# JoernZheng/parallel-data-compression-and-decompression

Hardware: NVIDIA B200
Metric: deflate/inflate GB/s (uncompressed) (higher is better)
Workload: dtype u8

## Files before the change

### parallel-data-compression-and-decompression_b200/csrc/deflate_match.cuh

```cuda
#pragma once
#include "zwz_common.cuh"

namespace zwz {

#define ZWZ_DM_NIL 0xffffu
#ifndef ZWZ_DM_NOISE_BITS
#define ZWZ_DM_NOISE_BITS 7.7f
#endif

#ifdef ZWZ_EMU
static uint64_t g_dm_stats[4];
extern "C" void zwz_emu_match_stats(uint64_t *out, int reset) {
    for (int i = 0; i < 4; ++i) {
        out[i] = g_dm_stats[i];
        if (reset) g_dm_stats[i] = 0;
    }
}
#define ZWZ_DM_STAT(i, v) do { g_dm_stats[i] += (v); } while (0)
#else
#define ZWZ_DM_STAT(i, v) do { } while (0)
#endif

template <int CLS> struct MatchClass;
template <> struct MatchClass<0> {
    static constexpr uint32_t kCap = 8192, kThreads = 256, kHBits = 12, kData = 8192 + 64, kListBits = 3, kCtasPerSm = 6;
    static constexpr uint32_t kPrevBytes = ((kCap + 31u) & ~31u) * 2u, kSmem = kData + kPrevBytes + (2u << kHBits) + 1024u + 2u * 8u * 8u;
};
template <> struct MatchClass<1> {
    static constexpr uint32_t kCap = 16384, kThreads = 512, kHBits = 13, kData = 16384 + 64, kListBits = 4, kCtasPerSm = 3;
    static constexpr uint32_t kPrevBytes = ((kCap + 31u) & ~31u) * 2u, kSmem = kData + kPrevBytes + (2u << kHBits) + 1024u + 2u * 16u * 16u;
};
template <> struct MatchClass<2> {
    static constexpr uint32_t kCap = 31744, kThreads = 512, kHBits = 13, kData = 31744 + 64, kListBits = 4, kCtasPerSm = 2;
    static constexpr uint32_t kPrevBytes = ((kCap + 31u) & ~31u) * 2u, kSmem = kData + kPrevBytes + (2u << kHBits) + 1024u + 2u * 16u * 16u;
};
template <> struct MatchClass<3> {
    static constexpr uint32_t kCap = 65535, kThreads = 1024, kHBits = 14, kData = 65600, kListBits = 5, kCtasPerSm = 1;
    static constexpr uint32_t kPrevBytes = ((kCap + 31u) & ~31u) * 2u, kSmem = kData + kPrevBytes + (2u << kHBits) + 640u + 2u * 32u * 32u;
};

struct MatchCtl {
    unsigned long long mbar;
    uint32_t next_tile;
    uint32_t cur_work;
    uint32_t nmatch;
    uint32_t skip[2];
    uint32_t coll;
    uint32_t coll2;
    uint32_t set2;
    uint32_t base[33];
    uint32_t adler_a[32], adler_b[32], adler_len[32];
};
static_assert(sizeof(MatchCtl) <= 640, "MatchCtl must fit its slot");
static_assert(MatchClass<0>::kPrevBytes >= (2u << MatchClass<0>::kHBits) && MatchClass<1>::kPrevBytes >= (2u << MatchClass<1>::kHBits) &&
                  MatchClass<2>::kPrevBytes >= (2u << MatchClass<2>::kHBits) && MatchClass<3>::kPrevBytes >= (2u << MatchClass<3>::kHBits),
              "the second bit set of the noise test lives in prev[]");
static_assert(2u * (MatchClass<2>::kSmem + 1024u) <= 228u * 1024u && 3u * (MatchClass<1>::kSmem + 1024u) <= 228u * 1024u &&
                  6u * (MatchClass<0>::kSmem + 1024u) <= 228u * 1024u,
              "resident CTAs per SM assumed by the launch grids");

ZWZ_DEV uint32_t dm_scratch_match_words(uint32_t n) { return scr_match_words(n); }

template <int HBITS> ZWZ_DEV uint32_t dm_hash3(uint32_t b0, uint32_t b1, uint32_t b2) {
    uint32_t v = b0 | (b1 << 8) | (b2 << 16);
    return (v * 0x9E3779B1u) >> (32 - HBITS);
}

#ifndef ZWZ_EMU
ZWZ_DEV uint32_t dm_smem_addr(const void *p) { return (uint32_t) __cvta_generic_to_shared(p); }
ZWZ_DEV void dm_mbar_init(unsigned long long *bar) {
    asm volatile("mbarrier.init.shared::cta.b64 [%0], 1;" ::"r"(dm_smem_addr(bar)));
    asm volatile("fence.mbarrier_init.release.cluster;" ::: "memory");
}
ZWZ_DEV void dm_bulk_g2s(void *dst, const void *src, uint32_t bytes, unsigned long long *bar) {
    asm volatile("fence.proxy.async.shared::cta;" ::: "memory");
    asm volatile("mbarrier.arrive.expect_tx.shared::cta.b64 _, [%0], %1;" ::"r"(dm_smem_addr(bar)), "r"(bytes) : "memory");
    asm volatile("cp.async.bulk.shared::cluster.global.mbarrier::complete_tx::bytes [%0], [%1], %2, [%3];" ::"r"(dm_smem_addr(dst)),
                 "l"(src), "r"(bytes), "r"(dm_smem_addr(bar))
                 : "memory");
}
ZWZ_DEV void dm_mbar_wait(unsigned long long *bar, uint32_t parity) {
    uint32_t done = 0;
    while (!done) {
        asm volatile("{\n\t.reg .pred p;\n\tmbarrier.try_wait.parity.shared::cta.b64 p, [%1], %2;\n\tselp.u32 %0, 1, 0, p;\n\t}"
                     : "=r"(done)
                     : "r"(dm_smem_addr(bar)), "r"(parity)
                     : "memory");
    }
}
#endif

ZWZ_DEV uint32_t sD_of(const unsigned char *smem, uint32_t skew) { return smem_addr(smem) + skew; }

template <int CLS, bool DICT = false>
ZWZ_KERNEL __launch_bounds__(MatchClass<CLS>::kThreads, MatchClass<CLS>::kCtasPerSm) lz_match_kernel(DeflateJob job, const uint32_t *__restrict__ order, uint32_t n_work,
                                                                         uint32_t *work_counter) {
    constexpr uint32_t T = MatchClass<CLS>::kThreads, HB = MatchClass<CLS>::kHBits, DATA = MatchClass<CLS>::kData;
    constexpr uint32_t NW = T / 32u, LB = MatchClass<CLS>::kListBits;
    static_assert((1u << LB) == NW, "one position list per warp");
    ZWZ_DYN_SMEM(smem);
    const uint32_t *dataw = (const uint32_t *) smem;
    uint16_t *prev = (uint16_t *) (smem + DATA);
    uint16_t *head = (uint16_t *) (smem + DATA + MatchClass<CLS>::kPrevBytes);
    MatchCtl *ctl = (MatchCtl *) (smem + DATA + MatchClass<CLS>::kPrevBytes + (2u << HB));
    uint16_t *cnt = (uint16_t *) ((unsigned char *) ctl + 640);
    const uint8_t *datab = (const uint8_t *) smem;
    const unsigned tid = threadIdx.x, lane = lane_id(), wid = warp_id();
    const unsigned lt = (1u << lane) - 1u;
    uint32_t parity = 0;

#ifndef ZWZ_EMU
    if (tid == 0) dm_mbar_init(&ctl->mbar);
#endif
    __syncthreads();

    for (;;) {
        if (tid == 0) ctl->cur_work = atomicAdd(work_counter, 1u);
        __syncthreads();
        const uint32_t w = ctl->cur_work;
        if (w >= n_work) break;
        const uint32_t c = order[w];
        const uint32_t n = job.raw_len[c];
        const uint8_t *src = job.raw + job.raw_off[c];
        const uint32_t skew = (uint32_t) ((uintptr_t) src & 15u);
        const uint32_t stage_bytes = (skew + n + 15u) & ~15u;
        const uint8_t *drec = nullptr;
        uint32_t dwl = 0;
        if (DICT) {
            const uint32_t di = job.dict.idx[c];
            if (di != ZWZ_NO_DICT) {
                drec = job.dict.arena + (size_t) di * ZWZ_DICT_STRIDE;
                dwl = job.dict.wlen[di];
            }
        }

#ifndef ZWZ_EMU
        if (tid == 0 && stage_bytes) dm_bulk_g2s(smem, src - skew, stage_bytes, &ctl->mbar);
#else
        for (uint32_t i = tid; i < skew + n; i += T) smem[i] = i < skew ? 0 : src[i - skew];
#endif
        for (uint32_t i = tid; i < NW * NW / 2u; i += T) ((uint32_t *) cnt)[i] = 0u;
        if (tid == 0) {
            ctl->next_tile = 0;
            ctl->nmatch = 0;
            ctl->skip[0] = 0;
            ctl->skip[1] = 0;
        }
#ifndef ZWZ_EMU
        if (stage_bytes) dm_mbar_wait(&ctl->mbar, parity);
        parity ^= (stage_bytes != 0u);
#endif
        __syncthreads();
        if (tid < 32u) smem[skew + n + tid] = 0;

        {
            uint32_t *hist = (uint32_t *) head + wid * 256u;
            const uint32_t nfull = n >> 10;
            for (uint32_t kb = wid; kb < nfull; kb += NW) {
                const uint32_t w0 = (skew + (kb << 10)) >> 2;
                {
                    const uint32_t sv = dataw[w0 + 8u * lane] & 0x80808080u;
                    const uint32_t tops = (uint32_t) (__popc(__ballot_sync(ZWZ_FULL, sv & 0x80u)) + __popc(__ballot_sync(ZWZ_FULL, sv & 0x8000u)) +
                                                      __popc(__ballot_sync(ZWZ_FULL, sv & 0x800000u)) + __popc(__ballot_sync(ZWZ_FULL, sv & 0x80000000u)));
                    if (tops < 40u || tops > 88u) continue;
                }
#pragma unroll
                for (uint32_t j = 0; j < 8u; ++j) hist[lane + 32u * j] = 0u;
                __syncwarp();
#pragma unroll
                for (uint32_t j = 0; j < 8u; ++j) {
                    const uint32_t wv = dataw[w0 + lane + 32u * j];
                    atomicAdd(&hist[wv & 0xffu], 1u);
                    atomicAdd(&hist[(wv >> 8) & 0xffu], 1u);
                    atomicAdd(&hist[(wv >> 16) & 0xffu], 1u);
                    atomicAdd(&hist[wv >> 24], 1u);
                }
                __syncwarp();
                float sum = 0.f;
#pragma unroll
                for (uint32_t j = 0; j < 8u; ++j) {
                    const float cf = (float) hist[lane + 32u * j];
                    if (cf > 1.f) sum += cf * zwz_log2f(cf);
                }
#pragma unroll
                for (int d = 16; d > 0; d >>= 1) sum += __shfl_xor_sync(ZWZ_FULL, sum, d);
                if (lane == 0 && sum < (10.f - ZWZ_DM_NOISE_BITS) * 1024.f) atomicOr(&ctl->skip[kb >> 5], 1u << (kb & 31u));
                __syncwarp();
            }
            __syncthreads();
            const uint64_t cand = (uint64_t) ctl->skip[0] | ((uint64_t) ctl->skip[1] << 32);
            if (cand) {
                constexpr uint32_t BB = HB + 4u;
                uint32_t *bits = (uint32_t *) head;
                __syncthreads();
                uint32_t *bits2 = (uint32_t *) prev;
                for (uint32_t i = tid; i < (1u << BB) / 32u; i += T) {
                    bits[i] = 0u;
                    bits2[i] = 0u;
                }
                if (tid == 0) {
                    ctl->coll = 0;
                    ctl->coll2 = 0;
                    ctl->set2 = 0;
                }
                __syncthreads();
                uint32_t mine = 0;
                for (uint32_t st = wid; st < nfull * 32u; st += NW) {
                    if (!((cand >> (st >> 5)) & 1ull)) continue;
                    const uint32_t h = (lds32u(sD_of(smem, skew) + st * 32u + lane) * 0x9E3779B1u) >> (32u - BB);
                    const uint32_t old = atomicOr(&bits[h >> 5], 1u << (h & 31u));
                    mine += (uint32_t) __popc(__ballot_sync(ZWZ_FULL, (old >> (h & 31u)) & 1u));
                }
                if (lane == 0 && mine) atomicAdd(&ctl->coll, mine);
                __syncthreads();
                const uint32_t nh = n >= 3u ? n - 2u : 0u;
                uint32_t fresh = 0;
                for (uint32_t st = wid; st * 32u < nh; st += NW) {
                    if (st < nfull * 32u && ((cand >> (st >> 5)) & 1ull)) continue;
                    const uint32_t q = st * 32u + lane;
                    const uint32_t h = (lds32u(sD_of(smem, skew) + q) * 0x9E3779B1u) >> (32u - BB);
                    const uint32_t old2 = q < nh ? atomicOr(&bits2[h >> 5], 1u << (h & 31u)) : 0xffffffffu;
                    fresh += (uint32_t) __popc(__ballot_sync(ZWZ_FULL, !((old2 >> (h & 31u)) & 1u)));
                }
                if (lane == 0 && fresh) atomicAdd(&ctl->set2, fresh);
                __syncthreads();
                uint32_t hits = 0;
                for (uint32_t st = wid; st < nfull * 32u; st += NW) {
                    if (!((cand >> (st >> 5)) & 1ull)) continue;
                    const uint32_t h = (lds32u(sD_of(smem, skew) + st * 32u + lane) * 0x9E3779B1u) >> (32u - BB);
                    hits += (uint32_t) __popc(__ballot_sync(ZWZ_FULL, (bits2[h >> 5] >> (h & 31u)) & 1u));
                }
                if (lane == 0 && hits) atomicAdd(&ctl->coll2, hits);
                __syncthreads();
                const uint32_t nc = (uint32_t) __popcll((long long) cand) << 10;
                const uint32_t allowed = (uint32_t) (((uint64_t) nc * nc) >> (BB + 1u)) + (nc >> 6) + 48u;
                const uint32_t allowed2 = (uint32_t) (((uint64_t) ctl->set2 * nc) >> BB) + (nc >> 6) + 48u;
                if (tid == 0 && (ctl->coll > allowed || ctl->coll2 > allowed2)) {
                    ctl->skip[0] = 0;
                    ctl->skip[1] = 0;
                    ZWZ_DM_STAT(1, 1);
                }
            }
        }
        __syncthreads();
        for (uint32_t i = tid; i < (1u << HB) / 2u; i += T) ((uint32_t *) head)[i] = 0xffffffffu;
        const uint64_t skipmask = (uint64_t) ctl->skip[0] | ((uint64_t) ctl->skip[1] << 32);
        if (tid == 0) {
            ZWZ_DM_STAT(0, (uint64_t) __popcll((long long) skipmask));
            ZWZ_DM_STAT(2, 1);
        }
        __syncthreads();

        uint32_t *mout = job.scratch + job.scr_off[c];
        uint16_t *list = (uint16_t *) (mout + dm_scratch_match_words(n));
        const uint32_t nhash = n >= 3u ? n - 2u : 0u;
        const uint32_t ntiles = (n + 31u) >> 5;
        const uint32_t nsteps = (nhash + 31u) >> 5;
        const uint32_t spw = (nsteps + NW - 1u) / NW;

        const uint32_t sD = smem_addr(smem) + skew;
        const uint32_t sP = smem_addr(prev);
        const uint32_t sH = smem_addr(head);
        const uint32_t sC = smem_addr(cnt);
        const uint32_t sB = smem_addr(&ctl->base[0]);
        for (uint32_t st = wid * spw; st < (wid + 1u) * spw && st < nsteps; ++st) {
            if ((skipmask >> (st >> 5)) & 1ull) continue;
            const uint32_t p = st * 32u + lane;
            const bool valid = p < nhash;
            uint32_t h = 0;
            if (valid) {
                uint32_t v = lds32u(sD + p);
                h = dm_hash3<HB>(v & 0xffu, (v >> 8) & 0xffu, (v >> 16) & 0xffu);
                sts16(sP + 2u * p, h);
            }
            const uint32_t b = h >> (HB - LB);
            unsigned m = __ballot_sync(ZWZ_FULL, valid);
#pragma unroll
            for (uint32_t k = 0; k < LB; ++k) {
                unsigned v = __ballot_sync(ZWZ_FULL, (b >> k) & 1u);
                m &= ((b >> k) & 1u) ? v : ~v;
            }
            if (valid && (m >> lane) == 1u) sts16(sC + 2u * (wid * NW + b), lds16(sC + 2u * (wid * NW + b)) + (uint32_t) __popc(m));
            __syncwarp();
        }
        __syncthreads();
        if (wid == 0) {
            uint32_t run = 0;
            if (lane < NW) {
                for (uint32_t ww = 0; ww < NW; ++ww) {
                    uint32_t t = cnt[ww * NW + lane];
                    cnt[ww * NW + lane] = (uint16_t) run;
                    run += t;
                }
            }
            uint32_t incl = warp_incl_scan(run);
            if (lane < NW) ctl->base[lane] = incl - run;
            if (lane == NW - 1u) ctl->base[NW] = incl;
        }
        __syncthreads();
        for (uint32_t st = wid * spw; st < (wid + 1u) * spw && st < nsteps; ++st) {
            if ((skipmask >> (st >> 5)) & 1ull) continue;
            const uint32_t p = st * 32u + lane;
            const bool valid = p < nhash;
            const uint32_t h = valid ? lds16(sP + 2u * p) : 0u;
            const uint32_t b = h >> (HB - LB);
            unsigned m = __ballot_sync(ZWZ_FULL, valid);
#pragma unroll
            for (uint32_t k = 0; k < LB; ++k) {
                unsigned v = __ballot_sync(ZWZ_FULL, (b >> k) & 1u);
                m &= ((b >> k) & 1u) ? v : ~v;
            }
            if (valid) {
                uint32_t slot = lds32(sB + 4u * b) + lds16(sC + 2u * (wid * NW + b)) + (uint32_t) __popc(m & lt);
                list[slot] = (uint16_t) p;
            }
            __syncwarp();
            if (valid && (m >> lane) == 1u) sts16(sC + 2u * (wid * NW + b), lds16(sC + 2u * (wid * NW + b)) + (uint32_t) __popc(m));
            __syncwarp();
        }
        __threadfence_block();
        __syncthreads();

        {
            const uint32_t i_end = ctl->base[wid + 1u];
            uint32_t i0 = ctl->base[wid];
            uint32_t qn = (i0 + lane < i_end) ? (uint32_t) __ldcg(list + i0 + lane) : 0u;
            for (; i0 < i_end; i0 += 32u) {
                const bool valid = i0 + lane < i_end;
                const uint32_t q = qn;
                qn = (i0 + 32u + lane < i_end) ? (uint32_t) __ldcg(list + i0 + 32u + lane) : 0u;
                const uint32_t h = valid ? lds16(sP + 2u * q) : 0u;
                uint32_t old = ZWZ_DM_NIL;
                if (valid) old = lds16(sH + 2u * h);
                __syncwarp();
                if (valid) {
                    sts16(sP + 2u * q, old);
                    sts16(sH + 2u * h, q);
                }
                __syncwarp();
                uint32_t rb = valid ? lds16(sH + 2u * h) : q;
                unsigned rem = __ballot_sync(ZWZ_FULL, rb != q);
                while (rem) {
                    const int leader = __ffs((int) rem) - 1;
                    const uint32_t hl = __shfl_sync(ZWZ_FULL, h, leader);
                    const bool mine = valid && h == hl;
                    const unsigned same = __ballot_sync(ZWZ_FULL, mine);
                    const unsigned lower = same & lt;
                    const int from = (mine && lower) ? 31 - __clz((int) lower) : (int) lane;
                    const uint32_t qlow = __shfl_sync(ZWZ_FULL, q, from);
                    if (mine) {
                        if (lower) sts16(sP + 2u * q, qlow);
                        if ((same >> lane) == 1u) sts16(sH + 2u * h, q);
                    }
                    rem &= ~same;
                }
                __syncwarp();
            }
        }
        __syncthreads();
        {
            const uint32_t list_lines = (nhash * 2u + 127u) >> 7;
            for (uint32_t i = tid; i < list_lines; i += T) discard_l2_line((const unsigned char *) list + 128u * i);
        }
        uint32_t *tflags = (uint32_t *) cnt;
        for (uint32_t i = tid; i < ZWZ_SCR_FLAG_WORDS && i < NW * NW / 2u; i += T) tflags[i] = 0u;
        __syncthreads();

        for (;;) {
            uint32_t tile = 0;
            if (lane == 0) tile = atomicAdd(&ctl->next_tile, 1u);
            tile = __shfl_sync(ZWZ_FULL, tile, 0);
            if (tile >= ntiles) break;
            if ((skipmask >> (tile >> 5)) & 1ull) {
                if (lane == 0) atomicMax(&ctl->next_tile, ((tile >> 5) + 1u) << 5);
                continue;
            }

            const uint32_t p = tile * 32u + lane;
            uint32_t best_len = 2u, best_dist = 0u;
            uint32_t maxlen = 0u;
            if (p < nhash) {
                maxlen = (n - p) < ZWZ_MAX_MATCH ? (n - p) : ZWZ_MAX_MATCH;
                const uint32_t limit = p > ZWZ_MAX_DIST ? p - ZWZ_MAX_DIST : 0u;
                const uint32_t span = p - limit;
                uint32_t cand = lds16(sP + 2u * p);
                if ((cand - limit) < span || (DICT && dwl != 0u && p < ZWZ_MAX_DIST)) {
                    const uint32_t ap = sD + p;
                    const uint32_t ka = ap & ~3u, sa = (ap & 3u) * 8u;
                    const uint32_t a0 = lds32(ka), a1 = lds32(ka + 4u), a2 = lds32(ka + 8u), a3 = lds32(ka + 12u);
                    const uint32_t S0 = __funnelshift_r(a0, a1, sa), S1 = __funnelshift_r(a1, a2, sa), S2 = __funnelshift_r(a2, a3, sa);
                    uint32_t scan_end = (S0 >> 16) & 0xffu, scan_end1 = (S0 >> 8) & 0xffu;
                    uint32_t budget = job.depth;
                    for (; budget != 0u && (cand - limit) < span; --budget) {
                        const uint32_t ac = sD + cand;
                        const uint32_t nxt = lds16(sP + 2u * cand);
                        if (lds8(ac + best_len) == scan_end && lds8(ac + best_len - 1u) == scan_end1) {
                            const uint32_t kc = ac & ~3u, sc = (ac & 3u) * 8u;
                            const uint32_t c0 = lds32(kc), c1 = lds32(kc + 4u), c2 = lds32(kc + 8u), c3 = lds32(kc + 12u);
                            const uint32_t x0 = __funnelshift_r(c0, c1, sc) ^ S0, x1 = __funnelshift_r(c1, c2, sc) ^ S1,
                                           x2 = __funnelshift_r(c2, c3, sc) ^ S2;
                            uint32_t len;
                            if (x0) {
                                len = ((uint32_t) __ffs((int) x0) - 1u) >> 3;
                            } else if (x1) {
                                len = 4u + (((uint32_t) __ffs((int) x1) - 1u) >> 3);
                            } else if (x2) {
                                len = 8u + (((uint32_t) __ffs((int) x2) - 1u) >> 3);
                            } else {
                                len = 12u;
                                while (len < maxlen) {
                                    uint32_t y = lds32u(ac + len) ^ lds32u(ap + len);
                                    if (y) {
                                        len += ((uint32_t) __ffs((int) y) - 1u) >> 3;
                                        break;
                                    }
                                    len += 4u;
                                }
                            }
                            if (len > maxlen) len = maxlen;
                            if (len > best_len) {
                                best_len = len;
                                best_dist = p - cand;
                                if (len >= job.nice || len >= maxlen) break;
                                scan_end = lds8(ap + len);
                                scan_end1 = lds8(ap + len - 1u);
                            }
                        }
                        cand = nxt;
                    }
                    if (DICT && budget != 0u && best_len < job.nice && best_len < maxlen && dwl != 0u && p < ZWZ_MAX_DIST) {
                        const uint16_t *dhead = (const uint16_t *) (drec + ZWZ_DICT_HEAD), *dprev = (const uint16_t *) (drec + ZWZ_DICT_PREV);
                        const uint8_t *dwin = drec + ZWZ_DICT_WIN;
                        const uint32_t dlim = p + dwl > ZWZ_MAX_DIST ? p + dwl - ZWZ_MAX_DIST : 0u;
                        const uint32_t dspan = dwl - dlim;
                        uint32_t q = __ldg(dhead + dm_hash3<ZWZ_DICT_HBITS>(S0 & 0xffu, (S0 >> 8) & 0xffu, (S0 >> 16) & 0xffu));
                        for (; budget != 0u && (q - dlim) < dspan; --budget) {
                            const uint32_t nxt = __ldg(dprev + q);
                            const uint32_t dmax = dwl - q < maxlen ? dwl - q : maxlen;
                            if (best_len < dmax && __ldg(dwin + q + best_len) == scan_end && __ldg(dwin + q + best_len - 1u) == scan_end1) {
                                uint32_t len = 0;
                                while (len < dmax) {
                                    const uint32_t y = ld32u((const uint32_t *) dwin, q + len) ^ lds32u(ap + len);
                                    if (y) {
                                        len += ((uint32_t) __ffs((int) y) - 1u) >> 3;
                                        break;
                                    }
                                    len += 4u;
                                }
                                if (len > dmax) len = dmax;
                                if (len > best_len) {
                                    best_len = len;
                                    best_dist = p + dwl - q;
                                    if (len >= job.nice || len >= maxlen) break;
                                    scan_end = lds8(ap + len);
                                    scan_end1 = lds8(ap + len - 1u);
                                }
                            }
                            q = nxt;
                        }
                    }
                }
            }
            if (__any_sync(ZWZ_FULL, best_len >= 4u)) {
                uint32_t key = best_len >= 3u ? best_len + lane : 0u, kd = best_dist;
#pragma unroll
                for (int d = 1; d < 32; d <<= 1) {
                    const uint32_t ok = __shfl_up_sync(ZWZ_FULL, key, d), od = __shfl_up_sync(ZWZ_FULL, kd, d);
                    if (lane >= (unsigned) d && ok > key) {
                        key = ok;
                        kd = od;
                    }
                }
                if (key >= lane + 3u && key - lane > best_len && key - lane <= maxlen) {
                    best_len = key - lane;
                    best_dist = kd;
                }
            }
            if (best_len == 3u && best_dist > 4096u) best_len = 2u;
            const unsigned hit = __ballot_sync(ZWZ_FULL, best_len >= 3u);
            if (hit) {
                if (p < n) mout[p] = tok_make(lds8(sD + p), best_len >= 3u ? best_len : 0u, best_dist);
                if (lane == 0) {
                    atomicAdd(&ctl->nmatch, (uint32_t) __popc(hit));
                    atomicOr(&tflags[tile >> 5], 1u << (tile & 31u));
                }
            }
        }
        __syncthreads();
        {
            uint32_t *gflags = mout + scr_flag_offset(n);
            const uint32_t used = (ntiles + 31u) >> 5;
            for (uint32_t i = tid; i < ZWZ_SCR_FLAG_WORDS; i += T) gflags[i] = i < used ? tflags[i] : 0u;
        }

        {
            AdlerPart part;
            part.a = 0;
            part.b = 0;
            part.len = 0;
            const uint32_t nwords = (skew + n + 3u) >> 2;
            for (uint32_t j = tid; j < nwords; j += T) {
                uint32_t wv = dataw[j];
                const int pos0 = (int) (4u * j) - (int) skew;
                if (pos0 < 0) wv = pos0 <= -4 ? 0u : wv & (0xffffffffu << (8u * (uint32_t) (-pos0)));
                if (pos0 + 4 > (int) n) wv &= 0xffffffffu >> (8u * (uint32_t) (pos0 + 4 - (int) n));
                const uint32_t s4 = zwz_dp4a(wv, 0x01010101u), w4 = zwz_dp4a(wv, 0x03020100u);
                part.a += s4;
                part.b += (uint32_t) ((int) n - pos0) * s4 - w4;
            }
            part.b %= 65521u;
#pragma unroll
            for (int d = 1; d < 32; d <<= 1) {
                AdlerPart o;
                o.a = __shfl_down_sync(ZWZ_FULL, part.a, d);
                o.b = __shfl_down_sync(ZWZ_FULL, part.b, d);
                o.len = __shfl_down_sync(ZWZ_FULL, part.len, d);
                if ((lane & (2u * d - 1u)) == 0u) part = adler_combine(part, o);
            }
            if (lane == 0) {
                ctl->adler_a[wid] = part.a;
                ctl->adler_b[wid] = part.b;
                ctl->adler_len[wid] = part.len;
            }
            __syncthreads();
            if (wid == 0) {
                part.a = lane < NW ? ctl->adler_a[lane] : 0u;
                part.b = lane < NW ? ctl->adler_b[lane] : 0u;
                part.len = lane < NW ? ctl->adler_len[lane] : 0u;
#pragma unroll
                for (int d = 1; d < 32; d <<= 1) {
                    AdlerPart o;
                    o.a = __shfl_down_sync(ZWZ_FULL, part.a, d);
                    o.b = __shfl_down_sync(ZWZ_FULL, part.b, d);
                    o.len = __shfl_down_sync(ZWZ_FULL, part.len, d);
                    if ((lane & (2u * d - 1u)) == 0u) part = adler_combine(part, o);
                }
                if (lane == 0) {
                    uint32_t a = (1u + part.a) % 65521u;
                    uint32_t b = (n % 65521u + part.b) % 65521u;
                    job.adler[c] = (b << 16) | a;
                    job.nmatch[c] = ctl->nmatch;
                }
            }
        }
        __syncthreads();
    }
}

#define ZWZ_DICT_SMEM (2u * 32768u + (2u << ZWZ_DICT_HBITS))
ZWZ_KERNEL __launch_bounds__(1024) dict_chain_kernel(const uint8_t *__restrict__ data, const uint64_t *__restrict__ win_off,
                                                     const uint32_t *__restrict__ wlen, uint8_t *arena) {
    ZWZ_DYN_SMEM(smem);
    uint16_t *prev = (uint16_t *) smem;
    uint16_t *head = (uint16_t *) (smem + 2u * 32768u);
    const unsigned tid = threadIdx.x, lane = lane_id(), T = blockDim.x;
    const unsigned lt = (1u << lane) - 1u;
    const uint32_t k = blockIdx.x, W = wlen[k];
    const uint8_t *src = data + win_off[k];
    uint8_t *rec = arena + (size_t) k * ZWZ_DICT_STRIDE;
    const uint32_t nh = W >= 3u ? W - 2u : 0u;
    for (uint32_t i = tid; i < W + 64u; i += T) rec[ZWZ_DICT_WIN + i] = i < W ? src[i] : (uint8_t) 0;
    for (uint32_t i = tid; i < (1u << ZWZ_DICT_HBITS); i += T) head[i] = (uint16_t) ZWZ_DM_NIL;
    for (uint32_t q = tid; q < nh; q += T) prev[q] = (uint16_t) dm_hash3<ZWZ_DICT_HBITS>(src[q], src[q + 1u], src[q + 2u]);
    __syncthreads();
    if (tid < 32u) {
        for (uint32_t i0 = 0; i0 < nh; i0 += 32u) {
            const uint32_t q = i0 + lane;
            const bool valid = q < nh;
            const uint32_t h = valid ? prev[q] : 0u;
            const uint32_t old = valid ? head[h] : (uint32_t) ZWZ_DM_NIL;
            __syncwarp();
            if (valid) {
                prev[q] = (uint16_t) old;
                head[h] = (uint16_t) q;
            }
            __syncwarp();
            const uint32_t rb = valid ? head[h] : q;
            unsigned rem = __ballot_sync(ZWZ_FULL, rb != q);
            while (rem) {
                const int leader = __ffs((int) rem) - 1;
                const uint32_t hl = __shfl_sync(ZWZ_FULL, h, leader);
                const bool mine = valid && h == hl;
                const unsigned same = __ballot_sync(ZWZ_FULL, mine);
                const unsigned lower = same & lt;
                const int from = (mine && lower) ? 31 - __clz((int) lower) : (int) lane;
                const uint32_t qlow = __shfl_sync(ZWZ_FULL, q, from);
                if (mine) {
                    if (lower) prev[q] = (uint16_t) qlow;
                    if ((same >> lane) == 1u) head[h] = (uint16_t) q;
                }
                __syncwarp();
                rem &= ~same;
            }
            __syncwarp();
        }
    }
    __syncthreads();
    uint16_t *ghead = (uint16_t *) (rec + ZWZ_DICT_HEAD), *gprev = (uint16_t *) (rec + ZWZ_DICT_PREV);
    for (uint32_t i = tid; i < (1u << ZWZ_DICT_HBITS); i += T) ghead[i] = head[i];
    for (uint32_t q = tid; q < nh; q += T) gprev[q] = prev[q];
}

}
```

Baseline: 34.83.

## Compact non-skipped strides and remove barriers in deflate match kernel

Builds a compacted list of non-skipped 1KB strides so the hashing and list-scatter loops iterate only over active work. Per-warp bucket counts are computed with ballots instead of shared read-modify-write, and offsets are carried in registers via shuffles. Several __syncthreads are removed, match-count atomics are batched per warp, and the L2 discard and flag writeback are moved after the Adler pass. Optional clock-based phase profiling macros are also added. The reordering of barriers risks subtle races if any removed sync was load-bearing.

```diff
diff --git a/parallel-data-compression-and-decompression_b200/csrc/deflate_match.cuh b/parallel-data-compression-and-decompression_b200/csrc/deflate_match.cuh
--- a/parallel-data-compression-and-decompression_b200/csrc/deflate_match.cuh
+++ b/parallel-data-compression-and-decompression_b200/csrc/deflate_match.cuh
@@ -17,8 +17,31 @@
     }
 }
 #define ZWZ_DM_STAT(i, v) do { g_dm_stats[i] += (v); } while (0)
+static uint64_t g_dm_skip[1u << 16];
+extern "C" void zwz_emu_match_skipmasks(uint64_t *out, uint32_t n) {
+    for (uint32_t i = 0; i < n && i < (1u << 16); ++i) out[i] = g_dm_skip[i];
+}
+#define ZWZ_DM_SKIP(c, m) do { if ((c) < (1u << 16)) g_dm_skip[c] = (m); } while (0)
 #else
 #define ZWZ_DM_STAT(i, v) do { } while (0)
+#define ZWZ_DM_SKIP(c, m) do { } while (0)
+#endif
+
+#define ZWZ_DM_NPHASE 10
+#if defined(ZWZ_DM_PHASE_CLOCKS) && !defined(ZWZ_EMU)
+__device__ unsigned long long g_dm_phase_clk[4][ZWZ_DM_NPHASE + 1];
+extern "C" int zwz_dm_phase_clocks(unsigned long long *out, int reset) {
+    if (cudaDeviceSynchronize() != cudaSuccess || cudaMemcpyFromSymbol(out, g_dm_phase_clk, sizeof(g_dm_phase_clk)) != cudaSuccess) return 1;
+    static const unsigned long long zero[4][ZWZ_DM_NPHASE + 1] = {};
+    return reset && cudaMemcpyToSymbol(g_dm_phase_clk, zero, sizeof(zero)) != cudaSuccess ? 1 : 0;
+}
+#define ZWZ_DM_CLK_DECL uint32_t dm_clk[ZWZ_DM_NPHASE + 1] = {}; long long dm_t0 = clock64();
+#define ZWZ_DM_CLK(k) do { if (tid == 0) { const long long t = clock64(); dm_clk[k] += (uint32_t) (t - dm_t0); dm_clk[ZWZ_DM_NPHASE] += (k == 0); dm_t0 = t; } } while (0)
+#define ZWZ_DM_CLK_FLUSH() do { if (tid == 0) for (int k = 0; k <= ZWZ_DM_NPHASE; ++k) atomicAdd(&g_dm_phase_clk[CLS][k], (unsigned long long) dm_clk[k]); } while (0)
+#else
+#define ZWZ_DM_CLK_DECL
+#define ZWZ_DM_CLK(k) do { } while (0)
+#define ZWZ_DM_CLK_FLUSH() do { } while (0)
 #endif
 
 template <int CLS> struct MatchClass;
@@ -41,14 +64,15 @@
 
 struct MatchCtl {
     unsigned long long mbar;
+    uint32_t cur_work;
     uint32_t next_tile;
-    uint32_t cur_work;
     uint32_t nmatch;
     uint32_t skip[2];
     uint32_t coll;
     uint32_t coll2;
     uint32_t set2;
     uint32_t base[33];
+    uint8_t slist[64];
     uint32_t adler_a[32], adler_b[32], adler_len[32];
 };
 static_assert(sizeof(MatchCtl) <= 640, "MatchCtl must fit its slot");
@@ -113,12 +137,16 @@
     if (tid == 0) dm_mbar_init(&ctl->mbar);
 #endif
     __syncthreads();
+    ZWZ_DM_CLK_DECL
 
     for (;;) {
         if (tid == 0) ctl->cur_work = atomicAdd(work_counter, 1u);
         __syncthreads();
         const uint32_t w = ctl->cur_work;
-        if (w >= n_work) break;
+        if (w >= n_work) {
+            ZWZ_DM_CLK_FLUSH();
+            break;
+        }
         const uint32_t c = order[w];
         const uint32_t n = job.raw_len[c];
         const uint8_t *src = job.raw + job.raw_off[c];
@@ -139,7 +167,6 @@
 #else
         for (uint32_t i = tid; i < skew + n; i += T) smem[i] = i < skew ? 0 : src[i - skew];
 #endif
-        for (uint32_t i = tid; i < NW * NW / 2u; i += T) ((uint32_t *) cnt)[i] = 0u;
         if (tid == 0) {
             ctl->next_tile = 0;
             ctl->nmatch = 0;
@@ -151,8 +178,10 @@
         parity ^= (stage_bytes != 0u);
 #endif
         __syncthreads();
+        ZWZ_DM_CLK(0);
         if (tid < 32u) smem[skew + n + tid] = 0;
 
+        uint64_t cand, skipmask;
         {
             uint32_t *hist = (uint32_t *) head + wid * 256u;
             const uint32_t nfull = n >> 10;
@@ -188,11 +217,12 @@
                 __syncwarp();
             }
             __syncthreads();
-            const uint64_t cand = (uint64_t) ctl->skip[0] | ((uint64_t) ctl->skip[1] << 32);
+            ZWZ_DM_CLK(1);
+            cand = (uint64_t) ctl->skip[0] | ((uint64_t) ctl->skip[1] << 32);
+            skipmask = cand;
             if (cand) {
                 constexpr uint32_t BB = HB + 4u;
                 uint32_t *bits = (uint32_t *) head;
-                __syncthreads();
                 uint32_t *bits2 = (uint32_t *) prev;
                 for (uint32_t i = tid; i < (1u << BB) / 32u; i += T) {
                     bits[i] = 0u;
@@ -204,122 +234,145 @@
                     ctl->set2 = 0;
                 }
                 __syncthreads();
+                const uint32_t sD0 = sD_of(smem, skew);
                 uint32_t mine = 0;
-                for (uint32_t st = wid; st < nfull * 32u; st += NW) {
-                    if (!((cand >> (st >> 5)) & 1ull)) continue;
-                    const uint32_t h = (lds32u(sD_of(smem, skew) + st * 32u + lane) * 0x9E3779B1u) >> (32u - BB);
-                    const uint32_t old = atomicOr(&bits[h >> 5], 1u << (h & 31u));
-                    mine += (uint32_t) __popc(__ballot_sync(ZWZ_FULL, (old >> (h & 31u)) & 1u));
+                for (uint64_t cm = cand; cm; cm &= cm - 1ull) {
+                    const uint32_t q0 = (uint32_t) (__ffsll((long long) cm) - 1) << 10;
+                    for (uint32_t j = wid; j < 32u; j += NW) {
+                        const uint32_t h = (lds32u(sD0 + q0 + j * 32u + lane) * 0x9E3779B1u) >> (32u - BB);
+                        const uint32_t old = atomicOr(&bits[h >> 5], 1u << (h & 31u));
+                        mine += (uint32_t) __popc(__ballot_sync(ZWZ_FULL, (old >> (h & 31u)) & 1u));
+                    }
                 }
                 if (lane == 0 && mine) atomicAdd(&ctl->coll, mine);
-                __syncthreads();
                 const uint32_t nh = n >= 3u ? n - 2u : 0u;
                 uint32_t fresh = 0;
-                for (uint32_t st = wid; st * 32u < nh; st += NW) {
-                    if (st < nfull * 32u && ((cand >> (st >> 5)) & 1ull)) continue;
-                    const uint32_t q = st * 32u + lane;
-                    const uint32_t h = (lds32u(sD_of(smem, skew) + q) * 0x9E3779B1u) >> (32u - BB);
-                    const uint32_t old2 = q < nh ? atomicOr(&bits2[h >> 5], 1u << (h & 31u)) : 0xffffffffu;
-                    fresh += (uint32_t) __popc(__ballot_sync(ZWZ_FULL, !((old2 >> (h & 31u)) & 1u)));
+                for (uint32_t q0 = 0; q0 < nh; q0 += 1024u) {
+                    if ((cand >> (q0 >> 10)) & 1ull) continue;
+                    for (uint32_t j = wid; j < 32u && q0 + j * 32u < nh; j += NW) {
+                        const uint32_t q = q0 + j * 32u + lane;
+                        const uint32_t h = (lds32u(sD0 + q) * 0x9E3779B1u) >> (32u - BB);
+                        const uint32_t old2 = q < nh ? atomicOr(&bits2[h >> 5], 1u << (h & 31u)) : 0xffffffffu;
+                        fresh += (uint32_t) __popc(__ballot_sync(ZWZ_FULL, !((old2 >> (h & 31u)) & 1u)));
+                    }
                 }
                 if (lane == 0 && fresh) atomicAdd(&ctl->set2, fresh);
                 __syncthreads();
                 uint32_t hits = 0;
-                for (uint32_t st = wid; st < nfull * 32u; st += NW) {
-                    if (!((cand >> (st >> 5)) & 1ull)) continue;
-                    const uint32_t h = (lds32u(sD_of(smem, skew) + st * 32u + lane) * 0x9E3779B1u) >> (32u - BB);
-                    hits += (uint32_t) __popc(__ballot_sync(ZWZ_FULL, (bits2[h >> 5] >> (h & 31u)) & 1u));
+                for (uint64_t cm = cand; cm; cm &= cm - 1ull) {
+                    const uint32_t q0 = (uint32_t) (__ffsll((long long) cm) - 1) << 10;
+                    for (uint32_t j = wid; j < 32u; j += NW) {
+                        const uint32_t h = (lds32u(sD0 + q0 + j * 32u + lane) * 0x9E3779B1u) >> (32u - BB);
+                        hits += (uint32_t) __popc(__ballot_sync(ZWZ_FULL, (bits2[h >> 5] >> (h & 31u)) & 1u));
+                    }
                 }
                 if (lane == 0 && hits) atomicAdd(&ctl->coll2, hits);
                 __syncthreads();
                 const uint32_t nc = (uint32_t) __popcll((long long) cand) << 10;
                 const uint32_t allowed = (uint32_t) (((uint64_t) nc * nc) >> (BB + 1u)) + (nc >> 6) + 48u;
                 const uint32_t allowed2 = (uint32_t) (((uint64_t) ctl->set2 * nc) >> BB) + (nc >> 6) + 48u;
-                if (tid == 0 && (ctl->coll > allowed || ctl->coll2 > allowed2)) {
-                    ctl->skip[0] = 0;
-                    ctl->skip[1] = 0;
-                    ZWZ_DM_STAT(1, 1);
-                }
-            }
-        }
-        __syncthreads();
+                if (ctl->coll > allowed || ctl->coll2 > allowed2) {
+                    skipmask = 0;
+                    if (tid == 0) ZWZ_DM_STAT(1, 1);
+                }
+            }
+        }
+        ZWZ_DM_CLK(2);
         for (uint32_t i = tid; i < (1u << HB) / 2u; i += T) ((uint32_t *) head)[i] = 0xffffffffu;
-        const uint64_t skipmask = (uint64_t) ctl->skip[0] | ((uint64_t) ctl->skip[1] << 32);
+        const uint32_t nstr = (n + 1023u) >> 10;
+        if (wid == 0) {
+#pragma unroll
+            for (uint32_t k = 0; k < 2u; ++k) {
+                const uint32_t sidx = 32u * k + lane;
+                const bool keep = sidx < nstr && !((skipmask >> sidx) & 1ull);
+                const unsigned km = __ballot_sync(ZWZ_FULL, keep);
+                if (keep) ctl->slist[(k ? (uint32_t) __popc((unsigned) ~skipmask) : 0u) + (uint32_t) __popc(km & lt)] = (uint8_t) sidx;
+            }
+        }
         if (tid == 0) {
             ZWZ_DM_STAT(0, (uint64_t) __popcll((long long) skipmask));
             ZWZ_DM_STAT(2, 1);
+            ZWZ_DM_SKIP(c, skipmask);
         }
         __syncthreads();
+        ZWZ_DM_CLK(3);
 
         uint32_t *mout = job.scratch + job.scr_off[c];
         uint16_t *list = (uint16_t *) (mout + dm_scratch_match_words(n));
         const uint32_t nhash = n >= 3u ? n - 2u : 0u;
-        const uint32_t ntiles = (n + 31u) >> 5;
-        const uint32_t nsteps = (nhash + 31u) >> 5;
+        const uint32_t nskip = 32u * (uint32_t) __popcll((long long) skipmask);
+        const uint32_t ntiles = ((n + 31u) >> 5) - nskip;
+        const uint32_t nsteps = ((nhash + 31u) >> 5) - nskip;
         const uint32_t spw = (nsteps + NW - 1u) / NW;
+        const uint32_t s_lo = wid * spw, s_hi = min(s_lo + spw, nsteps);
 
         const uint32_t sD = smem_addr(smem) + skew;
         const uint32_t sP = smem_addr(prev);
         const uint32_t sH = smem_addr(head);
-        const uint32_t sC = smem_addr(cnt);
-        const uint32_t sB = smem_addr(&ctl->base[0]);
-        for (uint32_t st = wid * spw; st < (wid + 1u) * spw && st < nsteps; ++st) {
-            if ((skipmask >> (st >> 5)) & 1ull) continue;
-            const uint32_t p = st * 32u + lane;
-            const bool valid = p < nhash;
-            uint32_t h = 0;
-            if (valid) {
-                uint32_t v = lds32u(sD + p);
-                h = dm_hash3<HB>(v & 0xffu, (v >> 8) & 0xffu, (v >> 16) & 0xffu);
-                sts16(sP + 2u * p, h);
-            }
-            const uint32_t b = h >> (HB - LB);
-            unsigned m = __ballot_sync(ZWZ_FULL, valid);
-#pragma unroll
-            for (uint32_t k = 0; k < LB; ++k) {
-                unsigned v = __ballot_sync(ZWZ_FULL, (b >> k) & 1u);
-                m &= ((b >> k) & 1u) ? v : ~v;
-            }
-            if (valid && (m >> lane) == 1u) sts16(sC + 2u * (wid * NW + b), lds16(sC + 2u * (wid * NW + b)) + (uint32_t) __popc(m));
-            __syncwarp();
+        const uint8_t *slist = ctl->slist;
+        {
+            uint32_t my = 0;
+            for (uint32_t i = s_lo; i < s_hi; ++i) {
+                const uint32_t p = (((uint32_t) slist[i >> 5] << 5) | (i & 31u)) * 32u + lane;
+                const bool valid = p < nhash;
+                uint32_t h = 0;
+                if (valid) {
+                    uint32_t v = lds32u(sD + p);
+                    h = dm_hash3<HB>(v & 0xffu, (v >> 8) & 0xffu, (v >> 16) & 0xffu);
+                    sts16(sP + 2u * p, h);
+                }
+                const uint32_t b = h >> (HB - LB);
+                unsigned ml = __ballot_sync(ZWZ_FULL, valid);
+#pragma unroll
+                for (uint32_t k = 0; k < LB; ++k) {
+                    const unsigned v = __ballot_sync(ZWZ_FULL, (b >> k) & 1u);
+                    ml &= ((lane >> k) & 1u) ? v : ~v;
+                }
+                my += (uint32_t) __popc(ml);
+            }
+            if (lane < NW) cnt[wid * NW + lane] = (uint16_t) my;
         }
         __syncthreads();
-        if (wid == 0) {
-            uint32_t run = 0;
+        ZWZ_DM_CLK(4);
+        uint32_t off;
+        {
+            uint32_t before = 0, total = 0;
             if (lane < NW) {
                 for (uint32_t ww = 0; ww < NW; ++ww) {
-                    uint32_t t = cnt[ww * NW + lane];
-                    cnt[ww * NW + lane] = (uint16_t) run;
-                    run += t;
-                }
-            }
-            uint32_t incl = warp_incl_scan(run);
-            if (lane < NW) ctl->base[lane] = incl - run;
-            if (lane == NW - 1u) ctl->base[NW] = incl;
-        }
-        __syncthreads();
-        for (uint32_t st = wid * spw; st < (wid + 1u) * spw && st < nsteps; ++st) {
-            if ((skipmask >> (st >> 5)) & 1ull) continue;
-            const uint32_t p = st * 32u + lane;
+                    const uint32_t t = cnt[ww * NW + lane];
+                    before += ww < wid ? t : 0u;
+                    total += t;
+                }
+            }
+            const uint32_t incl = warp_incl_scan(total);
+            off = incl - total + before;
+            if (wid == 0) {
+                if (lane < NW) ctl->base[lane] = incl - total;
+                if (lane == NW - 1u) ctl->base[NW] = incl;
+            }
+        }
+        ZWZ_DM_CLK(5);
+        for (uint32_t i = s_lo; i < s_hi; ++i) {
+            const uint32_t p = (((uint32_t) slist[i >> 5] << 5) | (i & 31u)) * 32u + lane;
             const bool valid = p < nhash;
             const uint32_t h = valid ? lds16(sP + 2u * p) : 0u;
             const uint32_t b = h >> (HB - LB);
-            unsigned m = __ballot_sync(ZWZ_FULL, valid);
+            unsigned m = __ballot_sync(ZWZ_FULL, valid), ml = m;
 #pragma unroll
             for (uint32_t k = 0; k < LB; ++k) {
-                unsigned v = __ballot_sync(ZWZ_FULL, (b >> k) & 1u);
+                const unsigned v = __ballot_sync(ZWZ_FULL, (b >> k) & 1u);
                 m &= ((b >> k) & 1u) ? v : ~v;
-            }
-            if (valid) {
-                uint32_t slot = lds32(sB + 4u * b) + lds16(sC + 2u * (wid * NW + b)) + (uint32_t) __popc(m & lt);
-                list[slot] = (uint16_t) p;
-            }
-            __syncwarp();
-            if (valid && (m >> lane) == 1u) sts16(sC + 2u * (wid * NW + b), lds16(sC + 2u * (wid * NW + b)) + (uint32_t) __popc(m));
-            __syncwarp();
+                ml &= ((lane >> k) & 1u) ? v : ~v;
+            }
+            const uint32_t o = __shfl_sync(ZWZ_FULL, off, b);
+            if (valid) list[o + (uint32_t) __popc(m & lt)] = (uint16_t) p;
+            off += (uint32_t) __popc(ml);
         }
         __threadfence_block();
         __syncthreads();
+        ZWZ_DM_CLK(6);
+        uint32_t *tflags = (uint32_t *) cnt;
+        for (uint32_t i = tid; i < ZWZ_SCR_FLAG_WORDS && i < NW * NW / 2u; i += T) tflags[i] = 0u;
 
         {
             const uint32_t i_end = ctl->base[wid + 1u];
@@ -358,146 +411,130 @@
             }
         }
         __syncthreads();
-        {
-            const uint32_t list_lines = (nhash * 2u + 127u) >> 7;
-            for (uint32_t i = tid; i < list_lines; i += T) discard_l2_line((const unsigned char *) list + 128u * i);
-        }
-        uint32_t *tflags = (uint32_t *) cnt;
-        for (uint32_t i = tid; i < ZWZ_SCR_FLAG_WORDS && i < NW * NW / 2u; i += T) tflags[i] = 0u;
-        __syncthreads();
-
+        ZWZ_DM_CLK(7);
+
+        uint32_t wmatch = 0;
         for (;;) {
-            uint32_t tile = 0;
-            if (lane == 0) tile = atomicAdd(&ctl->next_tile, 1u);
-            tile = __shfl_sync(ZWZ_FULL, tile, 0);
-            if (tile >= ntiles) break;
-            if ((skipmask >> (tile >> 5)) & 1ull) {
-                if (lane == 0) atomicMax(&ctl->next_tile, ((tile >> 5) + 1u) << 5);
-                continue;
-            }
-
-            const uint32_t p = tile * 32u + lane;
-            uint32_t best_len = 2u, best_dist = 0u;
-            uint32_t maxlen = 0u;
-            if (p < nhash) {
-                maxlen = (n - p) < ZWZ_MAX_MATCH ? (n - p) : ZWZ_MAX_MATCH;
-                const uint32_t limit = p > ZWZ_MAX_DIST ? p - ZWZ_MAX_DIST : 0u;
-                const uint32_t span = p - limit;
-                uint32_t cand = lds16(sP + 2u * p);
-                if ((cand - limit) < span || (DICT && dwl != 0u && p < ZWZ_MAX_DIST)) {
-                    const uint32_t ap = sD + p;
-                    const uint32_t ka = ap & ~3u, sa = (ap & 3u) * 8u;
-                    const uint32_t a0 = lds32(ka), a1 = lds32(ka + 4u), a2 = lds32(ka + 8u), a3 = lds32(ka + 12u);
-                    const uint32_t S0 = __funnelshift_r(a0, a1, sa), S1 = __funnelshift_r(a1, a2, sa), S2 = __funnelshift_r(a2, a3, sa);
-                    uint32_t scan_end = (S0 >> 16) & 0xffu, scan_end1 = (S0 >> 8) & 0xffu;
-                    uint32_t budget = job.depth;
-                    for (; budget != 0u && (cand - limit) < span; --budget) {
-                        const uint32_t ac = sD + cand;
-                        const uint32_t nxt = lds16(sP + 2u * cand);
-                        if (lds8(ac + best_len) == scan_end && lds8(ac + best_len - 1u) == scan_end1) {
-                            const uint32_t kc = ac & ~3u, sc = (ac & 3u) * 8u;
-                            const uint32_t c0 = lds32(kc), c1 = lds32(kc + 4u), c2 = lds32(kc + 8u), c3 = lds32(kc + 12u);
-                            const uint32_t x0 = __funnelshift_r(c0, c1, sc) ^ S0, x1 = __funnelshift_r(c1, c2, sc) ^ S1,
-                                           x2 = __funnelshift_r(c2, c3, sc) ^ S2;
-                            uint32_t len;
-                            if (x0) {
-                                len = ((uint32_t) __ffs((int) x0) - 1u) >> 3;
-                            } else if (x1) {
-                                len = 4u + (((uint32_t) __ffs((int) x1) - 1u) >> 3);
-                            } else if (x2) {
-                                len = 8u + (((uint32_t) __ffs((int) x2) - 1u) >> 3);
-                            } else {
-                                len = 12u;
-                                while (len < maxlen) {
-                                    uint32_t y = lds32u(ac + len) ^ lds32u(ap + len);
-                                    if (y) {
-                                        len += ((uint32_t) __ffs((int) y) - 1u) >> 3;
-                                        break;
+            uint32_t i = 0;
+            if (lane == 0) i = atomicAdd(&ctl->next_tile, 1u);
+            i = __shfl_sync(ZWZ_FULL, i, 0);
+            if (i >= ntiles) break;
+            const uint32_t tile = ((uint32_t) slist[i >> 5] << 5) | (i & 31u);
+                const uint32_t p = tile * 32u + lane;
+                uint32_t best_len = 2u, best_dist = 0u;
+                uint32_t maxlen = 0u;
+                if (p < nhash) {
+                    maxlen = (n - p) < ZWZ_MAX_MATCH ? (n - p) : ZWZ_MAX_MATCH;
+                    const uint32_t limit = p > ZWZ_MAX_DIST ? p - ZWZ_MAX_DIST : 0u;
+                    const uint32_t span = p - limit;
+                    uint32_t cand = lds16(sP + 2u * p);
+                    if ((cand - limit) < span || (DICT && dwl != 0u && p < ZWZ_MAX_DIST)) {
+                        const uint32_t ap = sD + p;
+                        const uint32_t ka = ap & ~3u, sa = (ap & 3u) * 8u;
+                        const uint32_t a0 = lds32(ka), a1 = lds32(ka + 4u), a2 = lds32(ka + 8u), a3 = lds32(ka + 12u);
+                        const uint32_t S0 = __funnelshift_r(a0, a1, sa), S1 = __funnelshift_r(a1, a2, sa), S2 = __funnelshift_r(a2, a3, sa);
+                        uint32_t scan_end = (S0 >> 16) & 0xffu, scan_end1 = (S0 >> 8) & 0xffu;
+                        uint32_t budget = job.depth;
+                        for (; budget != 0u && (cand - limit) < span; --budget) {
+                            const uint32_t ac = sD + cand;
+                            const uint32_t nxt = lds16(sP + 2u * cand);
+                            if (lds8(ac + best_len) == scan_end && lds8(ac + best_len - 1u) == scan_end1) {
+                                const uint32_t kc = ac & ~3u, sc = (ac & 3u) * 8u;
+                                const uint32_t c0 = lds32(kc), c1 = lds32(kc + 4u), c2 = lds32(kc + 8u), c3 = lds32(kc + 12u);
+                                const uint32_t x0 = __funnelshift_r(c0, c1, sc) ^ S0, x1 = __funnelshift_r(c1, c2, sc) ^ S1,
+                                               x2 = __funnelshift_r(c2, c3, sc) ^ S2;
+                                uint32_t len;
+                                if (x0) {
+                                    len = ((uint32_t) __ffs((int) x0) - 1u) >> 3;
+                                } else if (x1) {
+                                    len = 4u + (((uint32_t) __ffs((int) x1) - 1u) >> 3);
+                                } else if (x2) {
+                                    len = 8u + (((uint32_t) __ffs((int) x2) - 1u) >> 3);
+                                } else {
+                                    len = 12u;
+                                    while (len < maxlen) {
+                                        uint32_t y = lds32u(ac + len) ^ lds32u(ap + len);
+                                        if (y) {
+                                            len += ((uint32_t) __ffs((int) y) - 1u) >> 3;
+                                            break;
+                                        }
+                                        len += 4u;
                                     }
-                                    len += 4u;
                                 }
-                            }
-                            if (len > maxlen) len = maxlen;
-                            if (len > best_len) {
-                                best_len = len;
-                                best_dist = p - cand;
-                                if (len >= job.nice || len >= maxlen) break;
-                                scan_end = lds8(ap + len);
-                                scan_end1 = lds8(ap + len - 1u);
-                            }
-                        }
-                        cand = nxt;
-                    }
-                    if (DICT && budget != 0u && best_len < job.nice && best_len < maxlen && dwl != 0u && p < ZWZ_MAX_DIST) {
-                        const uint16_t *dhead = (const uint16_t *) (drec + ZWZ_DICT_HEAD), *dprev = (const uint16_t *) (drec + ZWZ_DICT_PREV);
-                        const uint8_t *dwin = drec + ZWZ_DICT_WIN;
-                        const uint32_t dlim = p + dwl > ZWZ_MAX_DIST ? p + dwl - ZWZ_MAX_DIST : 0u;
-                        const uint32_t dspan = dwl - dlim;
-                        uint32_t q = __ldg(dhead + dm_hash3<ZWZ_DICT_HBITS>(S0 & 0xffu, (S0 >> 8) & 0xffu, (S0 >> 16) & 0xffu));
-                        for (; budget != 0u && (q - dlim) < dspan; --budget) {
-                            const uint32_t nxt = __ldg(dprev + q);
-                            const uint32_t dmax = dwl - q < maxlen ? dwl - q : maxlen;
-                            if (best_len < dmax && __ldg(dwin + q + best_len) == scan_end && __ldg(dwin + q + best_len - 1u) == scan_end1) {
-                                uint32_t len = 0;
-                                while (len < dmax) {
-                                    const uint32_t y = ld32u((const uint32_t *) dwin, q + len) ^ lds32u(ap + len);
-                                    if (y) {
-                                        len += ((uint32_t) __ffs((int) y) - 1u) >> 3;
-                                        break;
-                                    }
-                                    len += 4u;
-                                }
-                                if (len > dmax) len = dmax;
+                                if (len > maxlen) len = maxlen;
                                 if (len > best_len) {
                                     best_len = len;
-                                    best_dist = p + dwl - q;
+                                    best_dist = p - cand;
                                     if (len >= job.nice || len >= maxlen) break;
                                     scan_end = lds8(ap + len);
                                     scan_end1 = lds8(ap + len - 1u);
                                 }
                             }
-                            q = nxt;
+                            cand = nxt;
+                        }
+                        if (DICT && budget != 0u && best_len < job.nice && best_len < maxlen && dwl != 0u && p < ZWZ_MAX_DIST) {
+                            const uint16_t *dhead = (const uint16_t *) (drec + ZWZ_DICT_HEAD), *dprev = (const uint16_t *) (drec + ZWZ_DICT_PREV);
+                            const uint8_t *dwin = drec + ZWZ_DICT_WIN;
+                            const uint32_t dlim = p + dwl > ZWZ_MAX_DIST ? p + dwl - ZWZ_MAX_DIST : 0u;
+                            const uint32_t dspan = dwl - dlim;
+                            uint32_t q = __ldg(dhead + dm_hash3<ZWZ_DICT_HBITS>(S0 & 0xffu, (S0 >> 8) & 0xffu, (S0 >> 16) & 0xffu));
+                            for (; budget != 0u && (q - dlim) < dspan; --budget) {
+                                const uint32_t nxt = __ldg(dprev + q);
+                                const uint32_t dmax = dwl - q < maxlen ? dwl - q : maxlen;
+                                if (best_len < dmax && __ldg(dwin + q + best_len) == scan_end && __ldg(dwin + q + best_len - 1u) == scan_end1) {
+                                    uint32_t len = 0;
+                                    while (len < dmax) {
+                                        const uint32_t y = ld32u((const uint32_t *) dwin, q + len) ^ lds32u(ap + len);
+                                        if (y) {
+                                            len += ((uint32_t) __ffs((int) y) - 1u) >> 3;
+                                            break;
+                                        }
+                                        len += 4u;
+                                    }
+                                    if (len > dmax) len = dmax;
+                                    if (len > best_len) {
+                                        best_len = len;
+                                        best_dist = p + dwl - q;
+                                        if (len >= job.nice || len >= maxlen) break;
+                                        scan_end = lds8(ap + len);
+                                        scan_end1 = lds8(ap + len - 1u);
+                                    }
+                                }
+                                q = nxt;
+                            }
                         }
                     }
                 }
-            }
-            if (__any_sync(ZWZ_FULL, best_len >= 4u)) {
-                uint32_t key = best_len >= 3u ? best_len + lane : 0u, kd = best_dist;
-#pragma unroll
-                for (int d = 1; d < 32; d <<= 1) {
-                    const uint32_t ok = __shfl_up_sync(ZWZ_FULL, key, d), od = __shfl_up_sync(ZWZ_FULL, kd, d);
-                    if (lane >= (unsigned) d && ok > key) {
-                        key = ok;
-                        kd = od;
+                if (__any_sync(ZWZ_FULL, best_len >= 4u)) {
+                    uint32_t key = best_len >= 3u ? best_len + lane : 0u, kd = best_dist;
+    #pragma unroll
+                    for (int d = 1; d < 32; d <<= 1) {
+                        const uint32_t ok = __shfl_up_sync(ZWZ_FULL, key, d), od = __shfl_up_sync(ZWZ_FULL, kd, d);
+                        if (lane >= (unsigned) d && ok > key) {
+                            key = ok;
+                            kd = od;
+                        }
                     }
-                }
-                if (key >= lane + 3u && key - lane > best_len && key - lane <= maxlen) {
-                    best_len = key - lane;
-                    best_dist = kd;
-                }
-            }
-            if (best_len == 3u && best_dist > 4096u) best_len = 2u;
-            const unsigned hit = __ballot_sync(ZWZ_FULL, best_len >= 3u);
-            if (hit) {
-                if (p < n) mout[p] = tok_make(lds8(sD + p), best_len >= 3u ? best_len : 0u, best_dist);
-                if (lane == 0) {
-                    atomicAdd(&ctl->nmatch, (uint32_t) __popc(hit));
-                    atomicOr(&tflags[tile >> 5], 1u << (tile & 31u));
-                }
-            }
-        }
-        __syncthreads();
+                    if (key >= lane + 3u && key - lane > best_len && key - lane <= maxlen) {
+                        best_len = key - lane;
+                        best_dist = kd;
+                    }
+                }
+                if (best_len == 3u && best_dist > 4096u) best_len = 2u;
+                const unsigned hit = __ballot_sync(ZWZ_FULL, best_len >= 3u);
+                if (hit) {
+                    if (p < n) mout[p] = tok_make(lds8(sD + p), best_len >= 3u ? best_len : 0u, best_dist);
+                    if (lane == 0) atomicOr(&tflags[tile >> 5], 1u << (tile & 31u));
+                    wmatch += (uint32_t) __popc(hit);
+                }
+        }
+        if (lane == 0 && wmatch) atomicAdd(&ctl->nmatch, wmatch);
+
+        AdlerPart part;
+        part.a = 0;
+        part.b = 0;
+        part.len = 0;
         {
-            uint32_t *gflags = mout + scr_flag_offset(n);
-            const uint32_t used = (ntiles + 31u) >> 5;
-            for (uint32_t i = tid; i < ZWZ_SCR_FLAG_WORDS; i += T) gflags[i] = i < used ? tflags[i] : 0u;
-        }
-
-        {
-            AdlerPart part;
-            part.a = 0;
-            part.b = 0;
-            part.len = 0;
             const uint32_t nwords = (skew + n + 3u) >> 2;
             for (uint32_t j = tid; j < nwords; j += T) {
                 uint32_t wv = dataw[j];
@@ -522,28 +559,38 @@
                 ctl->adler_b[wid] = part.b;
                 ctl->adler_len[wid] = part.len;
             }
-            __syncthreads();
-            if (wid == 0) {
-                part.a = lane < NW ? ctl->adler_a[lane] : 0u;
-                part.b = lane < NW ? ctl->adler_b[lane] : 0u;
-                part.len = lane < NW ? ctl->adler_len[lane] : 0u;
-#pragma unroll
-                for (int d = 1; d < 32; d <<= 1) {
-                    AdlerPart o;
-                    o.a = __shfl_down_sync(ZWZ_FULL, part.a, d);
-                    o.b = __shfl_down_sync(ZWZ_FULL, part.b, d);
-                    o.len = __shfl_down_sync(ZWZ_FULL, part.len, d);
-                    if ((lane & (2u * d - 1u)) == 0u) part = adler_combine(part, o);
-                }
-                if (lane == 0) {
-                    uint32_t a = (1u + part.a) % 65521u;
-                    uint32_t b = (n % 65521u + part.b) % 65521u;
-                    job.adler[c] = (b << 16) | a;
-                    job.nmatch[c] = ctl->nmatch;
-                }
-            }
         }
         __syncthreads();
+        ZWZ_DM_CLK(8);
+        {
+            const uint32_t list_lines = (nhash * 2u + 127u) >> 7;
+            for (uint32_t i = tid; i < list_lines; i += T) discard_l2_line((const unsigned char *) list + 128u * i);
+        }
+        {
+            uint32_t *gflags = mout + scr_flag_offset(n);
+            const uint32_t used = (((n + 31u) >> 5) + 31u) >> 5;
+            for (uint32_t i = tid; i < ZWZ_SCR_FLAG_WORDS; i += T) gflags[i] = i < used ? tflags[i] : 0u;
+        }
+        if (wid == 0) {
+            part.a = lane < NW ? ctl->adler_a[lane] : 0u;
+            part.b = lane < NW ? ctl->adler_b[lane] : 0u;
+            part.len = lane < NW ? ctl->adler_len[lane] : 0u;
+#pragma unroll
+            for (int d = 1; d < 32; d <<= 1) {
+                AdlerPart o;
+                o.a = __shfl_down_sync(ZWZ_FULL, part.a, d);
+                o.b = __shfl_down_sync(ZWZ_FULL, part.b, d);
+                o.len = __shfl_down_sync(ZWZ_FULL, part.len, d);
+                if ((lane & (2u * d - 1u)) == 0u) part = adler_combine(part, o);
+            }
+            if (lane == 0) {
+                uint32_t a = (1u + part.a) % 65521u;
+                uint32_t b = (n % 65521u + part.b) % 65521u;
+                job.adler[c] = (b << 16) | a;
+                job.nmatch[c] = ctl->nmatch;
+            }
+        }
+        ZWZ_DM_CLK(9);
     }
 }
 
```

Result: faster. 37.73, median of 6 (+8.3%).
